# liuzuxin/FSRL

Hardware: NVIDIA H100
Metric: env-steps/sec (collect+update) SafetyCarCircle-v0 PPO-Lag (higher is better)
Workload: dtype f32

## Files before the change

fsrl_b200/csrc/ppo_persist.cu:

```cuda
#include "ppo_persist.cuh"
#include "arena.cuh"
#include "ppo_loss.cuh"
#include "wgmma.cuh"
#include <cuda_pipeline.h>
#include <cstdlib>
#include <cmath>
#include <vector>

namespace fsrl {
namespace pp {

using namespace wg;

constexpr int WQ = 2;
constexpr int NEPI = 128 * WQ;
constexpr int TPB = NEPI + 32;
constexpr int C1 = 16 / WQ;
constexpr int C2 = 32 / WQ;
constexpr int RB = 64;
constexpr int MB = 256;
constexpr int KC = 32, NCH = 256 / KC;
constexpr int SLOT_BYTES = 32768, NSLOT = 4;
constexpr int A_CHUNK = 64 * KC * 4;
constexpr int ACC_LD = 68;
constexpr int OUTP = 8;
constexpr int H_ = 256;
constexpr int IMG = 65536;
enum { I_H1A_HI, I_H1A_LO, I_H1T_HI, I_H1T_LO, I_DZA_HI, I_DZA_LO, I_DZT_HI, I_DZT_LO, I_W2A_HI, I_W2A_LO, I_W2B_HI, I_W2B_LO, N_IMG };
constexpr int DB2P_OFF = N_IMG * IMG;
constexpr int DW3P_OFF = DB2P_OFF + 4 * H_;
constexpr int DB3P_OFF = DW3P_OFF + 4 * H_ * OUTP;
constexpr int MAXD = 40;
constexpr int XS_OFF = 2 * SLOT_BYTES;
static_assert(XS_OFF >= 2 * 32 * 65 * 2 * 4 && XS_OFF >= 2 * (MAXD + 1) * 64 * 4 &&
              XS_OFF + 128 * (MAXD + 1) * 4 <= NSLOT * SLOT_BYTES, "staged rows overlap the ring's scratch or dW1 partials");
constexpr int NSMAX = (MAXD + 1) * 32 + 32 + 32 * OUTP + 16;
constexpr int SLICE_OFF = DB3P_OFF + 4 * 16;
constexpr int NET_WS = SLICE_OFF + 8 * NSMAX;
constexpr int SUMSQ_FLOATS = 128;
constexpr int FLAG_LINE = 32;
constexpr int F_A = 0, F_C = 1, F_PER_NET = 2;
constexpr int TILE_PK = (64 * 64 / NEPI + 2) / 3;
constexpr int TILE_FLOATS = TILE_PK * NEPI * 4;
constexpr int SLICE_PK = (NSMAX + 2) / 3;
constexpr int XG_PER_NET = 16 * TILE_FLOATS + 8 * SLICE_PK * 4;
constexpr int MAX_MB = 16384;
constexpr long long WAIT_CYCLES = 6000000000LL;

struct Args {
    fsrl_ppo_update_t u;
    int n_mb, slot0;
    long long adam_t0;
    float* ws;
    unsigned* flags;
    int* err;
    const float* adam_tab;
    long long* dbg;
    int dbg_step;
    unsigned dp_seq;
    int dp_direct;
};
constexpr int DBG_CH = 48;
constexpr int DBG_N = DBG_CH + 2 * 3 * NCH;
#define STAMP(i) do { if (P.dbg && t == P.dbg_step) P.dbg[(size_t)blockIdx.x * DBG_N + (i)] = clock64(); } while (0)

struct AdamS { float w1, b2, w2, rbc2s, eps, neg_step; };
__device__ __forceinline__ float adam_one(float p, float g, float& m, float& v, const AdamS& a) {
    m = m + a.w1 * (g - m);
    v = v * a.b2 + (a.w2 * g) * g;
    const float sq = v > 0.f ? v * rsqrtf(v) : 0.f;
    const float denom = fmaf(sq, a.rbc2s, a.eps);
    return p + __fdividef(a.neg_step * m, denom);
}

__device__ __forceinline__ void fail(int* err, int code) {
    *reinterpret_cast<volatile int*>(err) = code;
    __threadfence_system();
    asm volatile("trap;");
}
__device__ __forceinline__ uint32_t pk_hash(float x, float y, float z) {
    const uint32_t a = __float_as_uint(x), b = __float_as_uint(y), c = __float_as_uint(z);
    return a ^ __funnelshift_l(b, b, 11) ^ __funnelshift_l(c, c, 22);
}
__device__ __forceinline__ bool pk_ok(const float4& v, uint32_t tag) { return (__float_as_uint(v.w) ^ pk_hash(v.x, v.y, v.z)) == tag; }
__device__ __forceinline__ void st_packet(float* p, float x, float y, float z, uint32_t tag) {
    asm volatile("st.relaxed.sys.global.v4.f32 [%0], {%1,%2,%3,%4};" ::"l"(p), "f"(x), "f"(y), "f"(z), "f"(__uint_as_float(tag ^ pk_hash(x, y, z))) : "memory");
}
__device__ __forceinline__ float4 ld_packet(const float* p) {
    float4 v;
    asm volatile("ld.relaxed.sys.global.v4.f32 {%0,%1,%2,%3}, [%4];" : "=f"(v.x), "=f"(v.y), "=f"(v.z), "=f"(v.w) : "l"(p) : "memory");
    return v;
}

__device__ __noinline__ float3 dp_gather(const float* src, long long stride, int me, int world, uint32_t tag,
                                        float ox, float oy, float oz, int* err, int code) {
    const long long t0w = clock64();
    float ax = 0.f, ay = 0.f, az = 0.f;
    for (int r0 = 0; r0 < world; r0 += 4) {
        float4 v[4];
        bool ok;
        do {
            ok = true;
#pragma unroll
            for (int k = 0; k < 4; ++k)
                if (r0 + k < world && r0 + k != me) v[k] = ld_packet(src + (size_t)(r0 + k) * stride);
#pragma unroll
            for (int k = 0; k < 4; ++k)
                if (r0 + k < world && r0 + k != me) ok = ok && pk_ok(v[k], tag);
            if (!ok && clock64() - t0w > 4 * WAIT_CYCLES) fail(err, code);
        } while (!ok);
#pragma unroll
        for (int k = 0; k < 4; ++k) {
            if (r0 + k >= world) continue;
            if (r0 + k == me) { ax += ox; ay += oy; az += oz; }
            else { ax += v[k].x; ay += v[k].y; az += v[k].z; }
        }
    }
    return make_float3(ax, ay, az);
}
__device__ __noinline__ void dp_push_all(const float* const* xg, size_t off, int me, int world, float x, float y, float z, uint32_t tag) {
    for (int r = 0; r < world; ++r)
        if (r != me) st_packet(const_cast<float*>(xg[r]) + off, x, y, z, tag);
}

// ... 96 lines not shown
                mma_m64n64k8_tf32(dm, ah, bh);
            }
        }
        wgmma_commit();
        if (j > 0) {
            wgmma_wait<1>();
            __syncwarp();
            if (lane < 8) mbar_arrive_cluster(empty_r + 8 * ((qq - 1) % NSLOT));
        }
    }
    wgmma_wait<0>();
    reg_fence(dm); reg_fence(dc);
    __syncwarp();
    if (lane < 8) mbar_arrive_cluster(empty_r + 8 * ((qq - 1) % NSLOT));
}
template <int N>
__device__ __forceinline__ void stage_acc(float* accs, const float (&dm)[N / 2], const float (&dc)[N / 2], int wq, int sp,
                                          int lane) {
    if (wq == 0) {
        const int r = 16 * sp + (lane >> 2);
#pragma unroll
        for (int i = 0; i < N / 8; ++i) {
            const int c = 8 * i + 2 * (lane & 3);
            *reinterpret_cast<float2*>(accs + r * ACC_LD + c) = make_float2(dm[4 * i] + dc[4 * i], dm[4 * i + 1] + dc[4 * i + 1]);
            *reinterpret_cast<float2*>(accs + (r + 8) * ACC_LD + c) =
                make_float2(dm[4 * i + 2] + dc[4 * i + 2], dm[4 * i + 3] + dc[4 * i + 3]);
        }
    }
    asm volatile("bar.sync %0, 64;" ::"r"(2 + sp) : "memory");
}

__device__ __forceinline__ void copy_operand(unsigned char* dst, const float* src, uint32_t bytes, uint64_t* bar, int g, int i,
                                             uint16_t cta_mask) {
    if (g == 1) {
        bulk_g2s(dst, src, bytes, bar);
        bulk_g2s(dst + bytes, src + IMG, bytes, bar);
        return;
    }
    const uint32_t piece = 2 * bytes / g, off = i * piece, part = off / bytes, in = off % bytes;
    bulk_g2s_multicast(dst + off, src + (size_t)part * IMG + in / 4, piece, bar, cta_mask);
}

template <int NC, int W>
__device__ __forceinline__ void transposed_stage(float* scr, const float (&hi)[NC], const float (&lo)[NC], int row, int c0) {
    constexpr int LO = W * 65;
#pragma unroll
    for (int j = 0; j < NC; ++j) {
        scr[(c0 + j) * 65 + row] = hi[j];
        scr[LO + (c0 + j) * 65 + row] = lo[j];
    }
}
template <int W>
__device__ __forceinline__ void transposed_flush(const float* scr, int et, float* img_hi, int row_base, int col_base) {
    constexpr int LO = W * 65;
    const int col = et % W;
    constexpr int GPT = 16 / (NEPI / W);
    const int g0 = (et / W) * GPT;
    float* dst = img_hi + (size_t)(row_base >> 2) * 256 + (size_t)(col_base + col) * 4;
#pragma unroll
    for (int q = 0; q < GPT; ++q) {
        const int g = g0 + q;
        const float* sh = scr + col * 65 + 4 * g;
        *reinterpret_cast<float4*>(dst + (size_t)g * 256) = make_float4(sh[0], sh[1], sh[2], sh[3]);
        *reinterpret_cast<float4*>(dst + IMG + (size_t)g * 256) = make_float4(sh[LO], sh[LO + 1], sh[LO + 2], sh[LO + 3]);
    }
}
template <int NC, int W>
__device__ __forceinline__ void store_transposed(float* scr, const float (&hi)[NC], const float (&lo)[NC], int row, int c0,
                                                 int et, float* img_hi, int row_base, int col_base) {
    transposed_stage<NC, W>(scr, hi, lo, row, c0);
    epi_bar();
    transposed_flush<W>(scr, et, img_hi, row_base, col_base);
    epi_bar();
}

__device__ __forceinline__ void stage_rows(float* xs, const float* obs, long long row0, int a, int D, int et) {
    const int i = et >> 1;
    const float* src = obs + (row0 + 64 * a + i + (i & 64)) * D;
    float* dst = xs + i * (D | 1);
    for (int d = et & 1; d < D; d += 2) __pipeline_memcpy_async(dst + d, src + d, 4);
    __pipeline_commit();
}

__device__ __forceinline__ float half_sum(float v) {
#pragma unroll
    for (int o = 8; o > 0; o >>= 1) v += __shfl_xor_sync(0xffffffffu, v, o);
    return v;
}

struct SliceMap {
    int w1, b2, w3, b3, n;
    __device__ __host__ SliceMap(int D) { w1 = 0; b2 = (D + 1) * 32; w3 = b2 + 32; b3 = w3 + 32 * OUTP; n = b3 + 16; }
};

struct DpCtx {
    const float* const* xg;
    long long region;
    int me, world;
    uint32_t tag;
    int* err;
    int direct;
};
__device__ __forceinline__ int dp_owner(int et, int q, int world) { return (int)((unsigned)((et >> 5) * TILE_PK + q) % (unsigned)world); }

__device__ __noinline__ void dp_tile_send(DpCtx d, size_t off, const float* accs, int trow, int cb2, int et) {
    float g[C2];
    acc_ld<C2>(accs, trow, cb2, g);
#pragma unroll
    for (int q = 0; q < TILE_PK; ++q) {
        const size_t o_q = (size_t)d.me * d.region + off + (size_t)q * NEPI * 4;
        const float x = g[3 * q], y = 3 * q + 1 < C2 ? g[3 * q + 1] : 0.f, z = 3 * q + 2 < C2 ? g[3 * q + 2] : 0.f;
        if (d.direct) {
            dp_push_all(d.xg, o_q, d.me, d.world, x, y, z, d.tag);
        } else {
            const int o = dp_owner(et, q, d.world);
            if (o != d.me) st_packet(const_cast<float*>(d.xg[o]) + o_q, x, y, z, d.tag);
        }
    }
}
__device__ __noinline__ void dp_tile_reduce(DpCtx d, size_t off, float* accs, int trow, int cb2, int et) {
    float g[C2];
    acc_ld<C2>(accs, trow, cb2, g);
    const float inv_world = 1.0f / (float)d.world;
    const float* loc = d.xg[d.me];
#pragma unroll
    for (int q = 0; q < TILE_PK; ++q) {
        if (dp_owner(et, q, d.world) != d.me) continue;
        const float3 s3 = dp_gather(loc + off + (size_t)q * NEPI * 4, d.region, d.me, d.world, d.tag, g[3 * q],
                                    3 * q + 1 < C2 ? g[3 * q + 1] : 0.f, 3 * q + 2 < C2 ? g[3 * q + 2] : 0.f, d.err, 41);
        const float ax = s3.x * inv_world, ay = s3.y * inv_world, az = s3.z * inv_world;
        dp_push_all(d.xg, (size_t)FSRL_P2P_MAX_RANKS * d.region + off + (size_t)q * NEPI * 4, d.me, d.world, ax, ay, az, d.tag);
        g[3 * q] = ax;
        if (3 * q + 1 < C2) g[3 * q + 1] = ay;
        if (3 * q + 2 < C2) g[3 * q + 2] = az;
    }
    acc_st<C2>(accs, trow, cb2, g);
}
__device__ __noinline__ float dp_tile_finish(DpCtx d, size_t off, float* accs, int trow, int cb2, int et) {
    float g[C2];
    const long long t0w = clock64();
    if (d.direct) {
        float own[C2];
        acc_ld<C2>(accs, trow, cb2, own);
#pragma unroll
        for (int jq = 0; jq < C2; ++jq) g[jq] = 0.f;
        for (int r = 0; r < d.world; ++r) {
            if (r == d.me) {
#pragma unroll
                for (int jq = 0; jq < C2; ++jq) g[jq] += own[jq];
                continue;
            }
            const float* src = d.xg[d.me] + (size_t)r * d.region + off;
            float4 v[TILE_PK];
            bool ok;
            do {
                ok = true;
#pragma unroll
                for (int q = 0; q < TILE_PK; ++q) v[q] = ld_packet(src + (size_t)q * NEPI * 4);
#pragma unroll
                for (int q = 0; q < TILE_PK; ++q) ok = ok && pk_ok(v[q], d.tag);
                if (!ok && clock64() - t0w > 4 * WAIT_CYCLES) fail(d.err, 42);
            } while (!ok);
#pragma unroll
            for (int q = 0; q < TILE_PK; ++q) {
                g[3 * q] += v[q].x;
                if (3 * q + 1 < C2) g[3 * q + 1] += v[q].y;
                if (3 * q + 2 < C2) g[3 * q + 2] += v[q].z;
            }
        }
        const float inv_world = 1.0f / (float)d.world;
        float sq = 0.f;
#pragma unroll
        for (int jq = 0; jq < C2; ++jq) { g[jq] *= inv_world; sq = fmaf(g[jq], g[jq], sq); }
        acc_st<C2>(accs, trow, cb2, g);
        return sq;
    }
    const float* res = d.xg[d.me] + (size_t)FSRL_P2P_MAX_RANKS * d.region + off;
    acc_ld<C2>(accs, trow, cb2, g);
    float4 v[TILE_PK];
    bool ok;
    do {
        ok = true;
#pragma unroll
        for (int q = 0; q < TILE_PK; ++q)
            if (dp_owner(et, q, d.world) != d.me) v[q] = ld_packet(res + (size_t)q * NEPI * 4);
#pragma unroll
        for (int q = 0; q < TILE_PK; ++q)
            if (dp_owner(et, q, d.world) != d.me) ok = ok && pk_ok(v[q], d.tag);
        if (!ok && clock64() - t0w > 4 * WAIT_CYCLES) fail(d.err, 42);
    } while (!ok);
    float sq = 0.f;
#pragma unroll
    for (int q = 0; q < TILE_PK; ++q) {
        if (dp_owner(et, q, d.world) == d.me) continue;
        g[3 * q] = v[q].x;
        if (3 * q + 1 < C2) g[3 * q + 1] = v[q].y;
        if (3 * q + 2 < C2) g[3 * q + 2] = v[q].z;
    }
#pragma unroll
    for (int jq = 0; jq < C2; ++jq) sq = fmaf(g[jq], g[jq], sq);
    acc_st<C2>(accs, trow, cb2, g);
    return sq;
}
__device__ __noinline__ void dp_slices(DpCtx d, size_t off_s, float* sp_g, int n, int et) {
    const int n3 = (n + 2) / 3;
    const float inv_world = 1.0f / (float)d.world;
    for (int i = et; i < n3; i += NEPI)
        dp_push_all(d.xg, (size_t)d.me * d.region + off_s + 4 * (size_t)i, d.me, d.world,
                    sp_g[3 * i], 3 * i + 1 < n ? sp_g[3 * i + 1] : 0.f, 3 * i + 2 < n ? sp_g[3 * i + 2] : 0.f, d.tag);
    const float* loc = d.xg[d.me];
    for (int i = et; i < n3; i += NEPI) {
        const float3 s3 = dp_gather(loc + off_s + 4 * (size_t)i, d.region, d.me, d.world, d.tag, sp_g[3 * i],
                                    3 * i + 1 < n ? sp_g[3 * i + 1] : 0.f, 3 * i + 2 < n ? sp_g[3 * i + 2] : 0.f, d.err, 40);
        sp_g[3 * i] = s3.x * inv_world;
        if (3 * i + 1 < n) sp_g[3 * i + 1] = s3.y * inv_world;
        if (3 * i + 2 < n) sp_g[3 * i + 2] = s3.z * inv_world;
    }
}

__device__ __forceinline__ bool red_cta() { return ((blockIdx.x >> 3) & 3) == ((blockIdx.x & 7) >> 2); }

__device__ __noinline__ float dp_tail(DpCtx d, size_t off_t, size_t off_s, float* accs, float* sp_g, int n, int trow, int cb2,
                                      int et, bool tile, bool slice) {
    if (tile && !d.direct) dp_tile_reduce(d, off_t, accs, trow, cb2, et);
    if (slice) dp_slices(d, off_s, sp_g, n, et);
    __syncwarp();
    return tile ? dp_tile_finish(d, off_t, accs, trow, cb2, et) : 0.f;
}

template <bool DP>
__global__ void __launch_bounds__(TPB, 1) ppo_persist_kernel(const Args P) {
    extern __shared__ __align__(1024) unsigned char smem_raw[];
    __shared__ __align__(8) uint64_t bar_full[NSLOT], bar_empty[NSLOT], bar_b, bar_w1;
    __shared__ float s_red[4][320];
    __shared__ float s_misc[32];
    __shared__ AdamS s_adam;
    __shared__ const float* s_xg[2][FSRL_P2P_MAX_RANKS];
    const fsrl_ppo_update_t& u = P.u;
    const int tid = threadIdx.x, warp = tid >> 5, lane = tid & 31;
    const int net = blockIdx.x >> 5, c = blockIdx.x & 31, a = c >> 3, b = c & 7;
    const bool is_g2 = c < 16;
    const int ka = (c & 15) >> 2, q4 = c & 3;

    const int D = u.D, A = u.A, C = u.C, H = H_;
    const int out = (net == 0) ? A : 1;
    const int n_cta = 32 * u.n_nets;
    float* wsn = P.ws + (size_t)net * NET_WS;
    float* sumsq_g = P.ws + (size_t)u.n_nets * NET_WS;
    unsigned* fl_net = P.flags + (size_t)net * F_PER_NET * FLAG_LINE;
    unsigned* fl_d2 = P.flags + (size_t)u.n_nets * F_PER_NET * FLAG_LINE;
    unsigned char* ring = smem_raw;
    float* accs = reinterpret_cast<float*>(smem_raw + NSLOT * SLOT_BYTES);
    float* small = accs + 64 * ACC_LD;
    const SliceMap sm(D);
    float* sp_p = small;
    float* sp_m = small + sm.n;
    float* sp_v = small + 2 * sm.n;
    float* sp_g = small + 3 * sm.n;
    float* land = small + 4 * sm.n;

    if (tid == 0) {
        for (int i = 0; i < NSLOT; ++i) { mbar_init(&bar_full[i], 1); mbar_init(&bar_empty[i], 4 * 8); }
        mbar_init(&bar_b, 1);
        mbar_init(&bar_w1, 4);
        fence_mbar_init();
    }
    __syncthreads();
    if (DP && threadIdx.x < 2 * FSRL_P2P_MAX_RANKS) s_xg[threadIdx.x / FSRL_P2P_MAX_RANKS][threadIdx.x % FSRL_P2P_MAX_RANKS] = P.u.p2p_xg[threadIdx.x / FSRL_P2P_MAX_RANKS][threadIdx.x % FSRL_P2P_MAX_RANKS];
    if (DP) __syncthreads();
    cluster_sync_all();

    const long long pbase = u.net_off[net];
    const ArenaLayout L = arena_layout(D, H, out, 0);
    const long long o_w1 = pbase + L.w1, o_b1 = pbase + L.b1, o_w2 = pbase + L.w2, o_b2 = pbase + L.b2,
                    o_w3 = pbase + L.w3, o_b3 = pbase + L.b3, o_ls = pbase + L.extra;

    if (warp == NEPI / 32) {
        if (elect_one()) {
            unsigned qq = 0;
            for (int t = 0; t < P.n_mb; ++t) {
                if (!flag_wait_ge<true>(fl_net + F_A * FLAG_LINE, 32u * (t + 1), WAIT_CYCLES)) fail(P.err, 10);
                STAMP(12);
                fence_proxy_async_global();
#pragma unroll 1
                for (int j = 0; j < NCH; ++j, ++qq) {
                    const int s = qq % NSLOT;
                    if (!mbar_wait(&bar_empty[s], ((qq / NSLOT) & 1) ^ 1, WAIT_CYCLES)) fail(P.err, 11);
#ifdef FSRL_PPO_CHUNK_STAMPS
                    STAMP(DBG_CH + j);
#endif
                    unsigned char* dst = ring + (size_t)s * SLOT_BYTES;
                    mbar_expect_tx(&bar_full[s], 3 * A_CHUNK);
                    const size_t ao = (size_t)a * 16384 + (size_t)j * 64 * KC, bo = (size_t)b * 8192 + (size_t)j * 32 * KC;
                    copy_operand(dst, wsn + (size_t)I_H1A_HI * IMG + ao, A_CHUNK, &bar_full[s], 8, b, 0xff);
                    copy_operand(dst + 2 * A_CHUNK, wsn + (size_t)I_W2A_HI * IMG + bo, A_CHUNK / 2, &bar_full[s], 1, 0, 0);
#ifdef FSRL_PPO_CHUNK_STAMPS
                    STAMP(DBG_CH + NCH + j);
#endif
                }
                STAMP(13);
                if (!flag_wait_ge<true>(fl_net + F_C * FLAG_LINE, 32u * (t + 1), WAIT_CYCLES)) fail(P.err, 12);
                STAMP(14);
                fence_proxy_async_global();
                const int ia = is_g2 ? I_W2B_HI : I_DZT_HI, ib = is_g2 ? I_DZA_HI : I_H1T_HI;
                const int blk_a = is_g2 ? ka : q4, blk_b = is_g2 ? q4 : ka;
                const uint16_t m4 = (uint16_t)(0xfu << (b & 4)), m2 = (uint16_t)(0x11u << (b & 3));
#pragma unroll 1
                for (int j = 0; j < NCH; ++j, ++qq) {
                    const int s = qq % NSLOT;
                    if (!mbar_wait(&bar_empty[s], ((qq / NSLOT) & 1) ^ 1, WAIT_CYCLES)) fail(P.err, 13);
#ifdef FSRL_PPO_CHUNK_STAMPS
                    STAMP(DBG_CH + 3 * NCH + j);
#endif
                    unsigned char* dst = ring + (size_t)s * SLOT_BYTES;
                    mbar_expect_tx(&bar_full[s], 4 * A_CHUNK);
                    const size_t ao = (size_t)blk_a * 16384 + (size_t)j * 64 * KC, bo = (size_t)blk_b * 16384 + (size_t)j * 64 * KC;
                    copy_operand(dst, wsn + (size_t)ia * IMG + ao, A_CHUNK, &bar_full[s], is_g2 ? 4 : 2, is_g2 ? b & 3 : b >> 2, is_g2 ? m4 : m2);
// ... 100 lines not shown
            if (is_g2) {
                const int r = et & 63, kc = C1 * (et >> 6);
                const float* x0 = xs + r * (D | 1);
                const float* x1 = xs + (64 + r) * (D | 1);
                float acc2[2][C1];
#pragma unroll
                for (int j = 0; j < C1; ++j) acc2[0][j] = acc2[1][j] = sp_p[sm.w1 + D * 32 + kc + j];
                for (int d = 0; d < D; ++d) {
                    const float xv0 = x0[d], xv1 = x1[d];
                    const float* w = sp_p + sm.w1 + d * 32 + kc;
#pragma unroll
                    for (int j = 0; j < C1; ++j) { acc2[0][j] = fmaf(xv0, w[j], acc2[0][j]); acc2[1][j] = fmaf(xv1, w[j], acc2[1][j]); }
                }
                constexpr int TSCR = 2 * 32 * 65;
#pragma unroll
                for (int rep = 0; rep < 2; ++rep) {
                    const int aa = a + 2 * rep;
                    float hi[C1], lo[C1];
                    float* a_hi = wsn + (size_t)I_H1A_HI * IMG + (size_t)aa * 16384 + (size_t)r * 4;
#pragma unroll
                    for (int q = 0; q < C1 / 4; ++q) {
#pragma unroll
                        for (int e = 0; e < 4; ++e) tf32_split(fmaxf(acc2[rep][4 * q + e], 0.f), hi[4 * q + e], lo[4 * q + e]);
                        const size_t plane = (size_t)(8 * b + (kc >> 2) + q) * 256;
                        *reinterpret_cast<float4*>(a_hi + plane) = make_float4(hi[4 * q], hi[4 * q + 1], hi[4 * q + 2], hi[4 * q + 3]);
                        *reinterpret_cast<float4*>(a_hi + IMG + plane) = make_float4(lo[4 * q], lo[4 * q + 1], lo[4 * q + 2], lo[4 * q + 3]);
                    }
                    transposed_stage<C1, 32>(scratch + rep * TSCR, hi, lo, r, kc);
                }
                epi_bar();
#pragma unroll
                for (int rep = 0; rep < 2; ++rep)
                    transposed_flush<32>(scratch + rep * TSCR, et, wsn + (size_t)I_H1T_HI * IMG + (size_t)(b >> 1) * 16384, 64 * (a + 2 * rep), 32 * (b & 1));
            }
            fence_proxy_async_smem();
            epi_bar();
            if (et == 0) { STAMP(1); flag_add_release(fl_net + F_A * FLAG_LINE); }

            const long long grow = row0 + 64 * a + trow;
            float p_act[8], p_lpo = 0.f, p_adv0 = 0.f, p_adv1 = 0.f, p_ret = 0.f, p_val = 0.f, mean[2] = {0.f, 0.f}, rstd[2] = {1.f, 1.f};
#pragma unroll
            for (int j = 0; j < 8; ++j) p_act[j] = 0.f;
            if (net == 0) {
#pragma unroll
                for (int j = 0; j < 8; ++j) if (j < A) p_act[j] = __ldg(u.act + grow * A + j);
                p_lpo = __ldg(u.logp_old + grow);
                p_adv0 = __ldg(u.adv + grow);
                if (C > 1) p_adv1 = __ldg(u.adv + u.ld + grow);
                const float* ms = u.mb_stats + (size_t)t * 4;
                mean[0] = __ldg(ms); rstd[0] = __ldg(ms + 1); mean[1] = __ldg(ms + 2); rstd[1] = __ldg(ms + 3);
            } else {
                p_ret = __ldg(u.ret + (long long)(net - 1) * u.ld + grow);
                if (u.value_clip) p_val = __ldg(u.values + (long long)(net - 1) * u.ld + grow);
            }
            float p_ls[8], p_rsg[8];
#pragma unroll
            for (int j = 0; j < 8; ++j) {
                p_ls[j] = (net == 0 && j < A) ? sp_p[sm.b3 + 8 + j] : 0.f;
                p_rsg[j] = 1.0f / expf(p_ls[j]);
            }

            {
                float dm[16], dc[16];
                if (wq == 0) gemm_phase<32>(ring, qq, bar_full, empty_r, dm, dc, P.err, 30, lane, P, t, 0);
                else qq += NCH;
                stage_acc<32>(accs, dm, dc, wq, sp, lane);
            }
            if (et == 0) STAMP(2);
            float h2[C1];
            acc_ld<C1>(accs, trow, cb1, h2);
            float hp[OUTP];
#pragma unroll
            for (int j = 0; j < OUTP; ++j) hp[j] = 0.f;
#pragma unroll
            for (int j = 0; j < C1; ++j) {
                h2[j] = fmaxf(h2[j] + sp_p[sm.b2 + cb1 + j], 0.f);
                const float* w = sp_p + sm.w3 + (cb1 + j) * OUTP;
#pragma unroll
                for (int jj = 0; jj < OUTP; ++jj) hp[jj] = fmaf(h2[j], w[jj], hp[jj]);
            }
#pragma unroll
            for (int jj = 0; jj < OUTP; ++jj) hp[jj] += __shfl_xor_sync(0xffffffffu, hp[jj], 16);
            if (WQ > 1) {
                float* xh = &s_red[0][0];
                if (half == 0 && wq > 0) {
#pragma unroll
                    for (int jj = 0; jj < OUTP; ++jj) xh[((wq - 1) * 64 + trow) * OUTP + jj] = hp[jj];
                }
                epi_bar();
                if (half == 0 && wq == 0) {
#pragma unroll
                    for (int w2 = 1; w2 < WQ; ++w2)
#pragma unroll
                        for (int jj = 0; jj < OUTP; ++jj) hp[jj] += xh[((w2 - 1) * 64 + trow) * OUTP + jj];
                }
            }
            float outv[OUTP];
#pragma unroll
            for (int jj = 0; jj < OUTP; ++jj) outv[jj] = sp_p[sm.b3 + jj];
            if (et == 0) {
                STAMP(3);
                mbar_expect_tx(&bar_b, 8u * 64u * OUTP * (uint32_t)sizeof(float));
            }
            if (half == 0 && wq == 0) {
                const uint32_t mine = smem_u32(land + ((size_t)b * 64 + trow) * OUTP);
                const uint32_t bb_ = smem_u32(&bar_b);
#pragma unroll
                for (int r = 0; r < 8; ++r) {
                    const uint32_t ra = mapa_u32(mine, r), rb = mapa_u32(bb_, r);
                    st_async4(ra, make_float4(hp[0], hp[1], hp[2], hp[3]), rb);
                    st_async4(ra + 16, make_float4(hp[4], hp[5], hp[6], hp[7]), rb);
                }
            }
            if (!mbar_wait_cluster(&bar_b, t & 1, WAIT_CYCLES)) fail(P.err, 31);
            __syncwarp();
            if (et == 0) STAMP(4);
#pragma unroll
            for (int bb = 0; bb < 8; ++bb) {
                const float* src = land + ((size_t)bb * 64 + trow) * OUTP;
                const float4 v0 = *reinterpret_cast<const float4*>(src);
                const float4 v1 = *reinterpret_cast<const float4*>(src + 4);
                outv[0] += v0.x; outv[1] += v0.y; outv[2] += v0.z; outv[3] += v0.w;
                outv[4] += v1.x; outv[5] += v1.y; outv[6] += v1.z; outv[7] += v1.w;
            }
            float dd[16];
#pragma unroll
            for (int j = 0; j < 16; ++j) dd[j] = 0.f;
            float st_a = 0.f, st_b = 0.f, st_c = 0.f, st_d = 0.f;
            {
                const float invB = 1.0f / (float)MB;
                if (net == 0) {
                    float g_mu[8], g_ls[8];
                    ppo_actor_row(u, outv, p_act, p_ls, p_rsg, p_lpo, p_adv0, p_adv1, mean, rstd, invB, g_mu, g_ls,
                                  st_a, st_b, st_c);
#pragma unroll
                    for (int j = 0; j < 8; ++j) { dd[j] = g_mu[j]; dd[8 + j] = g_ls[j]; }
                } else {
                    dd[0] = ppo_value_row(u, outv[0], p_ret, p_val, invB, st_d);
                }
            }
            if (et == 0) STAMP(26);
            const int nfeed = (net == 0) ? A : 1;
            float dz[C1];
#pragma unroll
            for (int j = 0; j < C1; ++j) {
                const float* w = sp_p + sm.w3 + (cb1 + j) * OUTP;
                float g = 0.f;
#pragma unroll
                for (int jj = 0; jj < OUTP; ++jj) if (jj < nfeed) g = fmaf(dd[jj], w[jj], g);
                dz[j] = h2[j] > 0.f ? g : 0.f;
            }
            {
                float hi[C1], lo[C1];
                float* a_hi = wsn + (size_t)I_DZA_HI * IMG + (size_t)a * 16384 + (size_t)trow * 4;
#pragma unroll
                for (int q = 0; q < C1 / 4; ++q) {
#pragma unroll
                    for (int e = 0; e < 4; ++e) tf32_split(dz[4 * q + e], hi[4 * q + e], lo[4 * q + e]);
                    const size_t plane = (size_t)(8 * b + (cb1 >> 2) + q) * 256;
                    *reinterpret_cast<float4*>(a_hi + plane) = make_float4(hi[4 * q], hi[4 * q + 1], hi[4 * q + 2], hi[4 * q + 3]);
                    *reinterpret_cast<float4*>(a_hi + IMG + plane) = make_float4(lo[4 * q], lo[4 * q + 1], lo[4 * q + 2], lo[4 * q + 3]);
                }
                store_transposed<C1, 32>(scratch, hi, lo, trow, cb1, et, wsn + (size_t)I_DZT_HI * IMG + (size_t)(b >> 1) * 16384, 64 * a, 32 * (b & 1));
            }
            if (et == 0) STAMP(27);
            {
                float* row = &s_red[sp][0];
#pragma unroll
                for (int j = 0; j < C1; ++j) {
                    const float sdz = half_sum(dz[j]);
                    if (r16 == 0) row[cb1 + j] = sdz;
                }
#pragma unroll
                for (int jj = 0; jj < OUTP; ++jj) {
                    if (jj < nfeed) {
#pragma unroll
                        for (int j = 0; j < C1; ++j) {
                            const float sv = half_sum(h2[j] * dd[jj]);
                            if (r16 == 0) row[32 + 32 * jj + cb1 + j] = sv;
                        }
                    }
                }
                if (b == 0 && wq == 0) {
#pragma unroll
                    for (int j = 0; j < 16; ++j) {
                        const float sv = half_sum(dd[j]);
                        if (lane == 0) row[288 + j] = sv;
                    }
                    const float sa = half_sum(st_a), sb = half_sum(st_b), sc = half_sum(st_c), sdv = half_sum(st_d);
                    if (lane == 0) { row[304] = sa; row[305] = sb; row[306] = sc; row[307] = sdv; }
                }
            }
            epi_bar();
            if (et == 0) STAMP(28);
            for (int i = et; i < 32 + 32 * nfeed; i += NEPI) {
                const float tot = ((s_red[0][i] + s_red[1][i]) + s_red[2][i]) + s_red[3][i];
                if (i < 32) wsn[DB2P_OFF + a * H + 32 * b + i] = tot;
                else wsn[DW3P_OFF + ((size_t)a * H + 32 * b + ((i - 32) & 31)) * OUTP + ((i - 32) >> 5)] = tot;
            }
            if (b == 0) {
                if (et < 20) {
                    const int i = 288 + et;
                    const float tot = ((s_red[0][i] + s_red[1][i]) + s_red[2][i]) + s_red[3][i];
                    if (et < 16) wsn[DB3P_OFF + a * 16 + et] = tot;
                    else {
                        float* stat = u.stats + (size_t)slot * FSRL_PPO_STATS;
                        if (net == 0) { if (et == 16) atomicAdd(stat + ST_ACTOR_REW, tot); if (et == 17) atomicAdd(stat + ST_ACTOR_SAFETY, tot); if (et == 18) atomicAdd(stat + ST_KL, tot); }
                        else if (et == 19) atomicAdd(stat + ST_VF0 + (net - 1), tot);
                    }
                }
                if (net == 0 && a == 0 && et == 20) u.stats[(size_t)slot * FSRL_PPO_STATS + ST_ENTROPY] = ppo_entropy(sp_p + sm.b3 + 8, A);
            }
            fence_proxy_async_smem();
            epi_bar();
            if (et == 0) { STAMP(5); flag_add_release(fl_net + F_C * FLAG_LINE); }

            unsigned mbits = 0;
            if (is_g2) {
                const int k = 64 * ka + trow;
                const float* msk = wsn + (size_t)I_H1A_HI * IMG + (size_t)q4 * 16384 + (size_t)(k >> 2) * 256 + (k & 3);
                float mreg[C2];
#pragma unroll
                for (int jq = 0; jq < C2; ++jq) mreg[jq] = __ldcg(msk + (size_t)(cb2 + jq) * 4);
                float xr[(64 * MAXD + NEPI - 1) / NEPI];
                const int nx = (64 * D + NEPI - 1) / NEPI;
                const float* xb = u.obs + (row0 + 64 * q4) * D;
#pragma unroll
                for (int q = 0; q < (64 * MAXD + NEPI - 1) / NEPI; ++q)
                    xr[q] = (q < nx && et + q * NEPI < 64 * D) ? __ldg(xb + et + q * NEPI) : 0.f;
#pragma unroll
                for (int jq = 0; jq < C2; ++jq) mbits |= (mreg[jq] > 0.f ? 1u : 0u) << jq;
#pragma unroll
                for (int q = 0; q < (64 * MAXD + NEPI - 1) / NEPI; ++q) {
                    const int e = et + q * NEPI;
                    if (q < nx && e < 64 * D) { const int r = e / D; land[r * ((D + 3) & ~3) + 4 * (r >> 5) + (e - r * D)] = xr[q]; }
                }
            }
            if (red_cta() && wq == 1) {
                const int tw = et - 128;
                if (tw == 0) {
                    if (!flag_wait_ge(fl_net + F_C * FLAG_LINE, 32u * (t + 1), WAIT_CYCLES)) fail(P.err, 35);
                    STAMP(15);
                }
                asm volatile("bar.sync 6, 128;" ::: "memory");
                for (int i0 = sm.b2 + tw; i0 < sm.n; i0 += 4 * 128) {
                    float pv[4][4];
#pragma unroll
                    for (int e = 0; e < 4; ++e) {
                        const int i = i0 + e * 128;
                        const float* src = wsn;
                        size_t stride = 0;
                        bool real = false;
                        if (i < sm.n) {
                            if (i < sm.w3) { src = wsn + DB2P_OFF + 32 * b + (i - sm.b2); stride = H; real = true; }
                            else if (i < sm.b3) {
                                const int oo = (i - sm.w3) / OUTP, jj = (i - sm.w3) % OUTP;
                                real = jj < out;
                                src = wsn + DW3P_OFF + ((size_t)32 * b + oo) * OUTP + jj; stride = (size_t)H * OUTP;
                            } else {
                                const int jj = i - sm.b3;
                                real = (jj < out) || (net == 0 && jj >= 8 && jj < 8 + A);
                                src = wsn + DB3P_OFF + jj; stride = 16;
                            }
                        }
#pragma unroll
                        for (int q = 0; q < 4; ++q) pv[e][q] = real ? __ldcg(src + q * stride) : 0.f;
                    }
#pragma unroll
                    for (int e = 0; e < 4; ++e) {
                        const int i = i0 + e * 128;
                        if (i < sm.n) {
                            float gsum = 0.f;
#pragma unroll
                            for (int q = 0; q < 4; ++q) gsum += pv[e][q];
                            sp_g[i] = gsum;
                        }
                    }
                }
                if (tw == 0) STAMP(16);
            }
            {
                float dm[32], dc[32];
                if (wq == 0) gemm_phase<64>(ring, qq, bar_full, empty_r, dm, dc, P.err, 32, lane, P, t, 1);
                else qq += NCH;
                stage_acc<64>(accs, dm, dc, wq, sp, lane);
            }
            if (et == 0) STAMP(6);
            float sq = 0.f;
            if (is_g2) {
                float v[C2];
                acc_ld<C2>(accs, trow, cb2, v);
#pragma unroll
                for (int jq = 0; jq < C2; ++jq) v[jq] = ((mbits >> jq) & 1u) ? v[jq] : 0.f;
                epi_bar();
                if (et == 0) STAMP(22);
                const int dp4 = (D + 3) & ~3;
                const float* xh = land + (size_t)cb2 * dp4 + 4 * half;
                float* dst = reinterpret_cast<float*>(ring) + (size_t)wq * (D + 1) * 64 + trow;
                for (int d0 = 0; d0 < D; d0 += 4) {
                    float sacc[4] = {0.f, 0.f, 0.f, 0.f};
#pragma unroll
                    for (int jq = 0; jq < C2; ++jq) {
                        const float4 x = *reinterpret_cast<const float4*>(xh + jq * dp4 + d0);
                        sacc[0] = fmaf(x.x, v[jq], sacc[0]);
                        sacc[1] = fmaf(x.y, v[jq], sacc[1]);
                        sacc[2] = fmaf(x.z, v[jq], sacc[2]);
                        sacc[3] = fmaf(x.w, v[jq], sacc[3]);
                    }
#pragma unroll
                    for (int i = 0; i < 4; ++i) sacc[i] += __shfl_xor_sync(0xffffffffu, sacc[i], 16);
                    if (half == 0) {
#pragma unroll
                        for (int i = 0; i < 4; ++i)
                            if (d0 + i < D) dst[(d0 + i) * 64] = sacc[i];
                    }
                }
                float sb1 = 0.f;
#pragma unroll
                for (int jq = 0; jq < C2; ++jq) sb1 += v[jq];
                sb1 += __shfl_xor_sync(0xffffffffu, sb1, 16);
                if (half == 0) dst[D * 64] = sb1;
                if (et == 0) STAMP(23);
                epi_bar();
                if (et == 0) mbar_arrive_release_cluster2(mapa_u32(smem_u32(&bar_w1), 2 * ka), mapa_u32(smem_u32(&bar_w1), 2 * ka + 1));
            } else {
                float g[C2];
                acc_ld<C2>(accs, trow, cb2, g);
                if (DP) {
                    dp_tile_send(dp_ctx(t), (size_t)(net * 16 + (c - 16)) * TILE_FLOATS + (size_t)et * 4, accs, trow, cb2, et);
                    if (et == 0) STAMP(32);
                } else {
#pragma unroll
                    for (int jq = 0; jq < C2; ++jq) sq = fmaf(g[jq], g[jq], sq);
                }
            }
            if (et == 0) STAMP(7);
            if (red_cta()) {
                if (!mbar_wait_cluster(&bar_w1, t & 1, WAIT_CYCLES)) fail(P.err, 33);
                if (et == 0) STAMP(8);
                const uint32_t ring_s = smem_u32(ring);
                const int kb = 32 * (b & 1);
                for (int i0 = et; i0 < sm.b2; i0 += 2 * NEPI) {
                    float pv[2][4 * WQ];
#pragma unroll
                    for (int e = 0; e < 2; ++e) {
                        const int i = i0 + e * NEPI;
                        const uint32_t off = 4u * (uint32_t)((i / 32) * 64 + kb + (i % 32));
#pragma unroll
                        for (int rb = 0; rb < 4; ++rb) {
                            const uint32_t src = mapa_u32(ring_s + off, (uint32_t)((4 * (b >> 1) + rb) & 7));
#pragma unroll
                            for (int w = 0; w < WQ; ++w)
                                pv[e][WQ * rb + w] = i < sm.b2 ? ld_cluster(src + 4u * (uint32_t)(w * (D + 1) * 64)) : 0.f;
                        }
                    }
#pragma unroll
                    for (int e = 0; e < 2; ++e) {
                        const int i = i0 + e * NEPI;
                        if (i < sm.b2) {
                            float gsum = 0.f;
#pragma unroll
                            for (int q = 0; q < 4 * WQ; ++q) gsum += pv[e][q];
                            sp_g[i] = gsum;
                        }
                    }
                }
                epi_bar();
// ... 12 lines not shown
                    bool real = true;
                    if (i >= sm.w3 && i < sm.b3) real = ((i - sm.w3) % OUTP) < out;
                    else if (i >= sm.b3) { const int jj = i - sm.b3; real = (jj < out) || (net == 0 && jj >= 8 && jj < 8 + A); }
                    if (real && (i < sm.b3 || b == 0)) sq = fmaf(sp_g[i], sp_g[i], sq);
                    wsn[SLICE_OFF + (size_t)b * NSMAX + i] = sp_g[i];
                }
            }
            if (red_cta() || !is_g2) {
                sq = warp_sum(sq);
                if (lane == 0) s_misc[warp] = sq;
                epi_bar();
                if (et == 0) {
                    float tot = 0.f;
#pragma unroll
                    for (int w2 = 0; w2 < NEPI / 32; ++w2) tot += s_misc[w2];
                    sumsq_g[blockIdx.x - (red_cta() ? 8 * a : 0)] = tot;
                    STAMP(9);
                    flag_add_release(fl_d2);
                }
            }
            if (is_g2 && t + 1 < P.n_mb) stage_rows(xs, u.obs, row0 + MB, a, D, et);
            if (et == 0) {
                if (!flag_wait_ge(fl_d2, 24u * (unsigned)u.n_nets * (t + 1), WAIT_CYCLES)) fail(P.err, 34);
                STAMP(10);
            }
            epi_bar();
            float nq[4];
#pragma unroll
            for (int q = 0; q < 4; ++q) nq[q] = (lane + 32 * q < n_cta) ? __ldcg(sumsq_g + lane + 32 * q) : 0.f;
            if (!DP && !red_cta())
                for (int i = et; i < sm.n; i += NEPI) sp_g[i] = __ldcg(wsn + SLICE_OFF + (size_t)b * NSMAX + i);
            float nsq = ((nq[0] + nq[1]) + nq[2]) + nq[3];
            nsq = warp_sum(nsq);
            float gscale = 1.0f;
            if (u.max_grad_norm > 0.f) gscale = fminf(u.max_grad_norm / (sqrtf(nsq) + 1e-6f), 1.0f);
            if (blockIdx.x == 0 && et == 0) u.stats[(size_t)slot * FSRL_PPO_STATS + ST_GRADNORM] = sqrtf(nsq);
            const AdamS ad = s_adam;
            if (et == 0) STAMP(24);
            for (int i = et; i < sm.n; i += NEPI) {
                float m = sp_m[i], v = sp_v[i];
                const float g = (DP && !red_cta()) ? __ldcg(wsn + SLICE_OFF + (size_t)b * NSMAX + i) : sp_g[i];
                sp_p[i] = adam_one(sp_p[i], g * gscale, m, v, ad);
                sp_m[i] = m; sp_v[i] = v;
            }
            if (et == 0) STAMP(25);
            if (!is_g2) {
                float g[C2];
                acc_ld<C2>(accs, trow, cb2, g);
#pragma unroll
                for (int j = 0; j < C2; ++j) w2p[j] = adam_one(w2p[j], g[j] * gscale, w2m[j], w2v[j], ad);
            } else {
                __pipeline_wait_prior(0);
                if (et == 0) STAMP(18);
            }
            epi_bar();
            if (et == 0) STAMP(11);
        }

        if (a == 0) {
            for (int i = et; i < sm.n; i += NEPI) {
                long long dst = -1;
                if (i < sm.b2) { const int d = i / 32, kk = i % 32; dst = (d < D) ? o_w1 + (long long)d * H + 32 * b + kk : o_b1 + 32 * b + kk; }
                else if (i < sm.w3) dst = o_b2 + 32 * b + (i - sm.b2);
                else if (i < sm.b3) { const int oo = (i - sm.w3) / OUTP, jj = (i - sm.w3) % OUTP; if (jj < out) dst = o_w3 + (long long)(32 * b + oo) * out + jj; }
                else if (b == 0) { const int jj = i - sm.b3; if (jj < out) dst = o_b3 + jj; else if (net == 0 && jj >= 8 && jj < 8 + A) dst = o_ls + (jj - 8); }
                if (dst >= 0) { u.theta[dst] = sp_p[i]; u.adam_m[dst] = sp_m[i]; u.adam_v[dst] = sp_v[i]; }
            }
        }
        if (!is_g2) {
            const int o = 64 * q4 + trow;
#pragma unroll
            for (int j = 0; j < C2; ++j) {
                const long long idx = o_w2 + (long long)(64 * ka + cb2 + j) * H + o;
                u.theta[idx] = w2p[j]; u.adam_m[idx] = w2m[j]; u.adam_v[idx] = w2v[j];
            }
        }
    }
    __syncthreads();
    cluster_sync_all();
}

static size_t smem_bytes(int D) {
    return (size_t)NSLOT * SLOT_BYTES + sizeof(float) * 64 * ACC_LD + 4 * sizeof(float) * SliceMap(D).n +
           sizeof(float) * 8 * 64 * OUTP;
}

static cudaLaunchConfig_t cluster_launch(int n_nets, size_t smem, cudaStream_t s, cudaLaunchAttribute* at) {
    at->id = cudaLaunchAttributeClusterDimension;
    at->val.clusterDim.x = 8; at->val.clusterDim.y = 1; at->val.clusterDim.z = 1;
    cudaLaunchConfig_t cfg = {};
    cfg.gridDim = dim3(32 * n_nets); cfg.blockDim = dim3(TPB); cfg.dynamicSmemBytes = smem; cfg.stream = s;
    cfg.attrs = at; cfg.numAttrs = 1;
    return cfg;
}

struct Instance {
    void (*kern)(const Args);
    int max_clusters;
};
static const Instance& instance(bool dp) {
    static Instance inst[2] = {};
    Instance& in = inst[dp];
    if (!in.kern) {
        in.kern = dp ? ppo_persist_kernel<true> : ppo_persist_kernel<false>;
        cudaLaunchAttribute at;
        const cudaLaunchConfig_t cfg = cluster_launch(1, smem_bytes(MAXD), nullptr, &at);
        if (cudaFuncSetAttribute(in.kern, cudaFuncAttributeMaxDynamicSharedMemorySize, (int)cfg.dynamicSmemBytes) != cudaSuccess ||
            cudaOccupancyMaxActiveClusters(&in.max_clusters, in.kern, &cfg) != cudaSuccess) {
            cudaGetLastError();
            in.max_clusters = 0;
        }
    }
    return in;
}

}

size_t ppo_persist_ws_floats(int n_nets, int D, int H) {
    (void)D; (void)H;
    return (size_t)n_nets * pp::NET_WS + pp::SUMSQ_FLOATS + (size_t)(n_nets * pp::F_PER_NET + 1) * pp::FLAG_LINE + 32 +
           2 * (size_t)pp::MAX_MB + 2 * (size_t)32 * n_nets * pp::DBG_N;
}

size_t ppo_persist_p2p_floats(int n_nets) { return (size_t)(FSRL_P2P_MAX_RANKS + 1) * n_nets * pp::XG_PER_NET + 64; }

bool ppo_persist_supported(const fsrl_ppo_update_t& u, long long n_total, int batch_size) {
    if (u.H != 256 || batch_size != pp::MB || n_total % pp::MB != 0 || n_total < pp::MB || n_total / pp::MB > pp::MAX_MB) return false;
    if (u.world > 1 && !(u.p2p_on && u.world <= FSRL_P2P_MAX_RANKS && (size_t)u.p2p_stride >= ppo_persist_p2p_floats(u.n_nets))) return false;
    if (u.D < 1 || u.D > pp::MAXD || u.A > 8 || u.n_nets < 1 || u.n_nets > 3) return false;
    if (u.persist_ws == nullptr || (size_t)u.persist_ws_floats < ppo_persist_ws_floats(u.n_nets, u.D, u.H)) return false;
    if (32 * u.n_nets > sm_count()) return false;
    return pp::instance(u.world > 1).max_clusters >= 4 * u.n_nets;
}

int ppo_persist_run(const fsrl_ppo_update_t& ug, int n_mb, int stats_slot0, long long adam_t0, cudaStream_t s) {
    pp::Args a;
    a.u = ug;
    a.n_mb = n_mb; a.slot0 = stats_slot0; a.adam_t0 = adam_t0;
    a.ws = ug.persist_ws;
    const size_t fl_off = (size_t)ug.n_nets * pp::NET_WS + pp::SUMSQ_FLOATS;
    a.flags = reinterpret_cast<unsigned*>(ug.persist_ws + fl_off);
    const size_t n_flag_words = (size_t)(ug.n_nets * pp::F_PER_NET + 1) * pp::FLAG_LINE;
    a.err = reinterpret_cast<int*>(a.flags + n_flag_words);
    FSRL_CUDA(cudaMemsetAsync(ug.persist_ws + fl_off - pp::SUMSQ_FLOATS, 0, (pp::SUMSQ_FLOATS + n_flag_words + 32) * sizeof(float), s));
    float* tab_dev = reinterpret_cast<float*>(a.err + 32);
    static std::vector<float> tab;
    tab.resize(2 * (size_t)n_mb);
    for (int t = 0; t < n_mb; ++t) {
        const double tt = (double)(adam_t0 + t + 1);
        const double bc1 = 1.0 - pow(ug.beta1, tt), bc2 = 1.0 - pow(ug.beta2, tt);
        tab[2 * t] = (float)(1.0 / sqrt(bc2));
        tab[2 * t + 1] = (float)(-(ug.lr / bc1));
    }
    FSRL_CUDA(cudaMemcpyAsync(tab_dev, tab.data(), tab.size() * sizeof(float), cudaMemcpyHostToDevice, s));
    a.adam_tab = tab_dev;
    static unsigned dp_seq = 0;
    if (ug.world > 1) dp_seq = (dp_seq % 65535u) + 1u;
    a.dp_seq = dp_seq;
    a.dp_direct = ug.world <= 2;
    if (const char* e = getenv("FSRL_PPO_DP_DIRECT")) a.dp_direct = atoi(e) != 0;
    a.dbg = nullptr; a.dbg_step = -1;
    if (const char* e = getenv("FSRL_PPO_PERSIST_DBG")) {
        a.dbg = reinterpret_cast<long long*>(tab_dev + 2 * (size_t)pp::MAX_MB);
        a.dbg_step = atoi(e);
    }
    cudaLaunchAttribute at;
    const cudaLaunchConfig_t cfg = pp::cluster_launch(ug.n_nets, pp::smem_bytes(ug.D), s, &at);
// ... 7 lines not shown
```

Measured before the change: 2.975 million.

## Move per-CTA dB2/dW3 column reductions to warpgroup 1 overlapping next GEMM

Replaces the shuffle-based half-warp reductions of dz and h2*dd, which every epilogue thread ran before signalling, with a column reduction done by the second epilogue warpgroup. That reduction reads dz/h2 staged in the accumulator buffer and row quantities staged in the landing buffer. The C flag is released earlier, and a new per-net flag F_P gates the reducer CTA's wait on these partials. Warpgroup 0 proceeds into the next GEMM phase, and named barriers 7 and 8 keep the accumulator buffer from being overwritten before the sums finish. This aims to take the reduction off the critical path, at the cost of an extra flag, extra barriers, and a changed summation order.

```diff
diff --git a/fsrl_b200/csrc/ppo_persist.cu b/fsrl_b200/csrc/ppo_persist.cu
--- a/fsrl_b200/csrc/ppo_persist.cu
+++ b/fsrl_b200/csrc/ppo_persist.cu
@@ -39,7 +39,10 @@
 constexpr int NET_WS = SLICE_OFF + 8 * NSMAX;
 constexpr int SUMSQ_FLOATS = 128;
 constexpr int FLAG_LINE = 32;
-constexpr int F_A = 0, F_C = 1, F_PER_NET = 2;
+constexpr int F_A = 0, F_C = 1, F_P = 2, F_PER_NET = 3;
+constexpr int LAND_FLOATS = 8 * 64 * OUTP;
+constexpr int ROWQ = 20, ROWQ_OFF = LAND_FLOATS - 64 * ROWQ;
+static_assert(63 * ((MAXD + 3) & ~3) + 4 + MAXD <= ROWQ_OFF, "G2's observation block overlaps the staged row quantities");
 constexpr int TILE_PK = (64 * 64 / NEPI + 2) / 3;
 constexpr int TILE_FLOATS = TILE_PK * NEPI * 4;
 constexpr int SLICE_PK = (NSMAX + 2) / 3;
@@ -302,10 +305,13 @@
     __pipeline_commit();
 }
 
-__device__ __forceinline__ float half_sum(float v) {
-#pragma unroll
-    for (int o = 8; o > 0; o >>= 1) v += __shfl_xor_sync(0xffffffffu, v, o);
-    return v;
+__device__ __forceinline__ float half_tree(const float (&v)[16]) {
+    float a8[8], a4[4];
+#pragma unroll
+    for (int l = 0; l < 8; ++l) a8[l] = v[l] + v[l + 8];
+#pragma unroll
+    for (int l = 0; l < 4; ++l) a4[l] = a8[l] + a8[l + 4];
+    return (a4[0] + a4[2]) + (a4[1] + a4[3]);
 }
 
 struct SliceMap {
@@ -452,7 +458,7 @@
 __global__ void __launch_bounds__(TPB, 1) ppo_persist_kernel(const Args P) {
     extern __shared__ __align__(1024) unsigned char smem_raw[];
     __shared__ __align__(8) uint64_t bar_full[NSLOT], bar_empty[NSLOT], bar_b, bar_w1;
-    __shared__ float s_red[4][320];
+    __shared__ float s_red[(WQ - 1) * 64 * OUTP];
     __shared__ float s_misc[32];
     __shared__ AdamS s_adam;
     __shared__ const float* s_xg[2][FSRL_P2P_MAX_RANKS];
@@ -719,7 +725,7 @@
 #pragma unroll
             for (int jj = 0; jj < OUTP; ++jj) hp[jj] += __shfl_xor_sync(0xffffffffu, hp[jj], 16);
             if (WQ > 1) {
-                float* xh = &s_red[0][0];
+                float* xh = s_red;
                 if (half == 0 && wq > 0) {
 #pragma unroll
                     for (int jj = 0; jj < OUTP; ++jj) xh[((wq - 1) * 64 + trow) * OUTP + jj] = hp[jj];
@@ -798,59 +804,61 @@
                     *reinterpret_cast<float4*>(a_hi + plane) = make_float4(hi[4 * q], hi[4 * q + 1], hi[4 * q + 2], hi[4 * q + 3]);
                     *reinterpret_cast<float4*>(a_hi + IMG + plane) = make_float4(lo[4 * q], lo[4 * q + 1], lo[4 * q + 2], lo[4 * q + 3]);
                 }
-                store_transposed<C1, 32>(scratch, hi, lo, trow, cb1, et, wsn + (size_t)I_DZT_HI * IMG + (size_t)(b >> 1) * 16384, 64 * a, 32 * (b & 1));
+                acc_st<C1>(accs, trow, cb1, dz);
+                acc_st<C1>(accs, trow, 32 + cb1, h2);
+                transposed_stage<C1, 32>(scratch, hi, lo, trow, cb1);
+                epi_bar();
+                if (wq == 0 && half == 0) {
+                    float4* rq = reinterpret_cast<float4*>(land + ROWQ_OFF + trow * ROWQ);
+#pragma unroll
+                    for (int q = 0; q < 4; ++q) rq[q] = make_float4(dd[4 * q], dd[4 * q + 1], dd[4 * q + 2], dd[4 * q + 3]);
+                    rq[4] = make_float4(st_a, st_b, st_c, st_d);
+                }
+                transposed_flush<32>(scratch, et, wsn + (size_t)I_DZT_HI * IMG + (size_t)(b >> 1) * 16384, 64 * a, 32 * (b & 1));
             }
             if (et == 0) STAMP(27);
-            {
-                float* row = &s_red[sp][0];
-#pragma unroll
-                for (int j = 0; j < C1; ++j) {
-                    const float sdz = half_sum(dz[j]);
-                    if (r16 == 0) row[cb1 + j] = sdz;
-                }
-#pragma unroll
-                for (int jj = 0; jj < OUTP; ++jj) {
-                    if (jj < nfeed) {
-#pragma unroll
-                        for (int j = 0; j < C1; ++j) {
-                            const float sv = half_sum(h2[j] * dd[jj]);
-                            if (r16 == 0) row[32 + 32 * jj + cb1 + j] = sv;
+            fence_proxy_async_smem();
+            epi_bar();
+            if (et == 0) { STAMP(19); flag_add_release(fl_net + F_C * FLAG_LINE); }
+
+            if (wq == 1) {
+                const int tw = et - 128;
+                const float* rq = land + ROWQ_OFF;
+                const int n_w3 = 32 + 32 * nfeed, n_el = n_w3 + (b == 0 ? ROWQ : 0);
+                for (int i = tw; i < n_el; i += 128) {
+                    const bool prod = i >= 32 && i < n_w3;
+                    const float* src = i < 32 ? accs + i : prod ? accs + 32 + ((i - 32) & 31) : rq + (i - n_w3);
+                    const float* ddp = rq + ((i - 32) >> 5);
+                    const int ld = i < n_w3 ? ACC_LD : ROWQ;
+                    float s[4];
+#pragma unroll
+                    for (int k = 0; k < 4; ++k) {
+                        float v[16];
+#pragma unroll
+                        for (int l = 0; l < 16; ++l) {
+                            const int r = 16 * k + l;
+                            v[l] = prod ? __fmul_rn(src[r * ld], ddp[r * ROWQ]) : src[r * ld];
+                        }
+                        s[k] = half_tree(v);
+                    }
+                    const float tot = ((s[0] + s[1]) + s[2]) + s[3];
+                    if (i < 32) wsn[DB2P_OFF + a * H + 32 * b + i] = tot;
+                    else if (prod) wsn[DW3P_OFF + ((size_t)a * H + 32 * b + ((i - 32) & 31)) * OUTP + ((i - 32) >> 5)] = tot;
+                    else {
+                        const int j = i - n_w3;
+                        if (j < 16) wsn[DB3P_OFF + a * 16 + j] = tot;
+                        else {
+                            float* stat = u.stats + (size_t)slot * FSRL_PPO_STATS;
+                            if (net == 0) { if (j == 16) atomicAdd(stat + ST_ACTOR_REW, tot); if (j == 17) atomicAdd(stat + ST_ACTOR_SAFETY, tot); if (j == 18) atomicAdd(stat + ST_KL, tot); }
+                            else if (j == 19) atomicAdd(stat + ST_VF0 + (net - 1), tot);
                         }
                     }
                 }
-                if (b == 0 && wq == 0) {
-#pragma unroll
-                    for (int j = 0; j < 16; ++j) {
-                        const float sv = half_sum(dd[j]);
-                        if (lane == 0) row[288 + j] = sv;
-                    }
-                    const float sa = half_sum(st_a), sb = half_sum(st_b), sc = half_sum(st_c), sdv = half_sum(st_d);
-                    if (lane == 0) { row[304] = sa; row[305] = sb; row[306] = sc; row[307] = sdv; }
-                }
-            }
-            epi_bar();
-            if (et == 0) STAMP(28);
-            for (int i = et; i < 32 + 32 * nfeed; i += NEPI) {
-                const float tot = ((s_red[0][i] + s_red[1][i]) + s_red[2][i]) + s_red[3][i];
-                if (i < 32) wsn[DB2P_OFF + a * H + 32 * b + i] = tot;
-                else wsn[DW3P_OFF + ((size_t)a * H + 32 * b + ((i - 32) & 31)) * OUTP + ((i - 32) >> 5)] = tot;
-            }
-            if (b == 0) {
-                if (et < 20) {
-                    const int i = 288 + et;
-                    const float tot = ((s_red[0][i] + s_red[1][i]) + s_red[2][i]) + s_red[3][i];
-                    if (et < 16) wsn[DB3P_OFF + a * 16 + et] = tot;
-                    else {
-                        float* stat = u.stats + (size_t)slot * FSRL_PPO_STATS;
-                        if (net == 0) { if (et == 16) atomicAdd(stat + ST_ACTOR_REW, tot); if (et == 17) atomicAdd(stat + ST_ACTOR_SAFETY, tot); if (et == 18) atomicAdd(stat + ST_KL, tot); }
-                        else if (et == 19) atomicAdd(stat + ST_VF0 + (net - 1), tot);
-                    }
-                }
-                if (net == 0 && a == 0 && et == 20) u.stats[(size_t)slot * FSRL_PPO_STATS + ST_ENTROPY] = ppo_entropy(sp_p + sm.b3 + 8, A);
-            }
-            fence_proxy_async_smem();
-            epi_bar();
-            if (et == 0) { STAMP(5); flag_add_release(fl_net + F_C * FLAG_LINE); }
+                if (net == 0 && a == 0 && b == 0 && tw == 127) u.stats[(size_t)slot * FSRL_PPO_STATS + ST_ENTROPY] = ppo_entropy(sp_p + sm.b3 + 8, A);
+                asm volatile("bar.arrive 8, %0;" ::"n"(NEPI) : "memory");
+                asm volatile("bar.sync 7, 128;" ::: "memory");
+                if (tw == 0) { STAMP(20); flag_add_release(fl_net + F_P * FLAG_LINE); }
+            }
 
             unsigned mbits = 0;
             if (is_g2) {
@@ -876,8 +884,8 @@
             if (red_cta() && wq == 1) {
                 const int tw = et - 128;
                 if (tw == 0) {
-                    if (!flag_wait_ge(fl_net + F_C * FLAG_LINE, 32u * (t + 1), WAIT_CYCLES)) fail(P.err, 35);
-                    STAMP(15);
+                    if (!flag_wait_ge(fl_net + F_P * FLAG_LINE, 32u * (t + 1), WAIT_CYCLES)) fail(P.err, 35);
+                    STAMP(21);
                 }
                 asm volatile("bar.sync 6, 128;" ::: "memory");
                 for (int i0 = sm.b2 + tw; i0 < sm.n; i0 += 4 * 128) {
@@ -918,8 +926,12 @@
             }
             {
                 float dm[32], dc[32];
-                if (wq == 0) gemm_phase<64>(ring, qq, bar_full, empty_r, dm, dc, P.err, 32, lane, P, t, 1);
-                else qq += NCH;
+                if (wq == 0) {
+                    gemm_phase<64>(ring, qq, bar_full, empty_r, dm, dc, P.err, 32, lane, P, t, 1);
+                    asm volatile("bar.sync 8, %0;" ::"n"(NEPI) : "memory");
+                } else {
+                    qq += NCH;
+                }
                 stage_acc<64>(accs, dm, dc, wq, sp, lane);
             }
             if (et == 0) STAMP(6);
@@ -1098,7 +1110,7 @@
 
 static size_t smem_bytes(int D) {
     return (size_t)NSLOT * SLOT_BYTES + sizeof(float) * 64 * ACC_LD + 4 * sizeof(float) * SliceMap(D).n +
-           sizeof(float) * 8 * 64 * OUTP;
+           sizeof(float) * LAND_FLOATS;
 }
 
 static cudaLaunchConfig_t cluster_launch(int n_nets, size_t smem, cudaStream_t s, cudaLaunchAttribute* at) {
```

After: 3.036 million, median of 6. 1.02x the previous value.
